# sydney-machine-learning/parallel-tempering-neural-net

Measured on AMD Instinct MI355X. Metric: MCMC samples/sec (all replicas) + swap-accept rate; Sunspot 64-replica FNN, higher is better.
Workload: dtype f32

## Files before the change

parallel-tempering-neural-net_amd/csrc/ptnn_dev_pack.hpp:

```cpp

constexpr int PK_WAVES = 8, PK_SWEEP_WAVES = 2, PK_FWD_WAVES = 4;
__host__ __device__ constexpr int pack_slots(int nred) { return PK_SWEEP_WAVES * (WAVE >> nred); }

__host__ __device__ inline size_t pack_slot_floats(int PS) { return 2 * (size_t)PS; }
__host__ __device__ inline size_t pack_ring_floats(int PS, int nslots) { return (size_t)2 * nslots * ((size_t)PS + 4); }
__host__ __device__ inline size_t pack_lds_floats(int Nall, int IPY, int PS, int H, int FWS, int nslots) {
    return (size_t)(Nall + 2) * IPY + 4 * (size_t)PS + MAX_WAVES * 8 + (size_t)nslots * SL_COUNT +
           (size_t)nslots * pack_slot_floats(PS) + pack_ring_floats(PS, nslots) + (size_t)PK_WAVES * fw_floats(H, FWS);
}
constexpr int PK_MULTI_MAXG = 4;
__host__ __device__ inline size_t pack_multi_lds_floats(int Nall, int IPY, int PS, int H, int FWS, int nslots) {
    return pack_lds_floats(Nall, IPY, PS, H, FWS, nslots) + pack_ring_floats(PS, (PK_MULTI_MAXG - 1) * nslots) + 2 * (size_t)PS + SL_COUNT + 8;
}

template <int TASK, int I, int O, int PK_NRED, bool MULTI = false>
__device__ __forceinline__ void segment_pack_body(const SegParams& p, const SegDyn& dyn, const int step_begin, const int n_steps) {
    constexpr int PK_NG = WAVE >> PK_NRED, PK_SLOTS = pack_slots(PK_NRED);
    extern __shared__ __attribute__((aligned(16))) float smem[];
    const int G = MULTI ? p.G : 1;
    const int lb = MULTI ? xcd_block(G) : (int)blockIdx.x;
    const int r = MULTI ? lb / G : lb, grp = MULTI ? lb - r * G : 0;
    const int KT = G * PK_SLOTS, s0 = grp * PK_SLOTS;
    const int gid = p.first_global + r;
    const int tid = threadIdx.x, nthr = blockDim.x;
    const int wave = tid >> 6, lane = tid & 63;
    const int Nall = p.Ntr + p.Nte;
    const int P = p.P, PS = p.PS, H = p.H;
    float* q = smem;
    float* xy = q; q += (Nall + 2) * p.IPY;
    float* w_cur = q; q += PS;
    float* w_gd = q; q += PS;
    float* rec_w = q; q += PS;
    float* rec_alt = q; q += PS;
    float* red = q; q += MAX_WAVES * 8;
    float* slots = q; q += PK_SLOTS * SL_COUNT;
    const size_t SLF = pack_slot_floats(PS);
    float* sl0 = q; q += PK_SLOTS * SLF;
    constexpr int RING = (MULTI ? 2 * PK_MULTI_MAXG : 2) * PK_SLOTS;
    float* ring_n = q; q += (size_t)RING * PS;
    float* ring_s = q; q += (size_t)RING * 4;
    float* my_fw = q + (size_t)wave * fw_floats(H, p.FWS);
    q += (size_t)PK_WAVES * fw_floats(H, p.FWS);
    float* win_v = q; q += MULTI ? 2 * (size_t)PS : 0;
    float* win_s = q; q += MULTI ? SL_COUNT : 0;
    float* gverd = q;
    granule_t* const xv = MULTI ? p.xverdict + (size_t)r * 2 * MAX_SLOTS : nullptr;
    granule_t* const xsl = MULTI ? p.xslots + (size_t)r * 2 * MAX_SLOTS * SL_COUNT : nullptr;
    granule_t* const xwv = MULTI ? p.xw + (size_t)r * 2 * G * 2 * PS : nullptr;
    unsigned epoch = dyn.epoch_base;
    int xpar = 0;
    bool failed = false;
    auto s_prop = [&](int s_) { return sl0 + (size_t)s_ * SLF; };
    auto s_pgd = [&](int s_) { return sl0 + (size_t)s_ * SLF + PS; };

    {
        const float4* src = reinterpret_cast<const float4*>(p.data);
        float4* dst = reinterpret_cast<float4*>(xy);
        for (int e = tid; e < ((Nall + 2) * p.IPY) >> 2; e += nthr) dst[e] = src[e];
    }
    float* gw = dyn.w_state + (size_t)r * PS;
    for (int j = tid; j < PS; j += nthr) {
        w_cur[j] = gw[j];
        rec_w[j] = p.rec_w[(size_t)r * PS + j];
        w_gd[j] = dyn.gd_w[(size_t)r * PS + j];
    }
    __syncthreads();

    const float T = uni_f(p.temps[r]);
    float eta = (TASK == TASK_REG) ? uni_f(w_cur[P]) : 0.0f;
    float* sf = p.st_f + (size_t)r * SF_COUNT;
    int* si = p.st_i + (size_t)r * SI_COUNT;
    float lik, prior_cur, tau_eta_last, rec_rmse_tr, rec_rmse_te, rec_acc_tr, rec_acc_te;
    int nacc, gd_valid, lg_count, lg_acc;
    if (step_begin == 0) {
        lg_acc = 0;
        if (wave == 0) {
            chain_startup<TASK, I, O, true>(p, xy, w_cur, my_fw, red, T, eta, lik, prior_cur);
            if (lane == 0) { red[0] = eta; red[1] = lik; red[2] = prior_cur; }
        }
        __syncthreads();
        eta = uni_f(red[0]); lik = uni_f(red[1]); prior_cur = uni_f(red[2]);
        tau_eta_last = eta;
        rec_rmse_tr = rec_rmse_te = rec_acc_tr = rec_acc_te = 0.f;
        nacc = 0; gd_valid = 0; lg_count = 0;
        __syncthreads();
    } else {
        lik = uni_f(sf[SF_LIK]); prior_cur = uni_f(sf[SF_PRIOR]); tau_eta_last = uni_f(sf[SF_TAU_LAST]);
        rec_rmse_tr = uni_f(sf[SF_REC_RMSE_TR]); rec_rmse_te = uni_f(sf[SF_REC_RMSE_TE]);
        rec_acc_tr = uni_f(sf[SF_REC_ACC_TR]); rec_acc_te = uni_f(sf[SF_REC_ACC_TE]);
        nacc = uni_i(si[SI_NACC]); gd_valid = uni_i(dyn.gd_valid[r]); lg_count = uni_i(si[SI_LG_COUNT]); lg_acc = uni_i(si[SI_LG_ACC]);
    }

    PTNN_DIAG(pack_begin);
    const size_t trow = (size_t)r * p.trace_cap;
    const int end = step_begin + n_steps;
    const bool sweeping = p.use_lg != 0;
    const int nwaves = nthr >> 6;
    const int ev_n = sweeping ? (nwaves == PK_WAVES ? PK_FWD_WAVES : 2) : nwaves;
    const int ev_i = !sweeping ? wave : ((wave & 3) >= 2 ? (wave & 1) + ((wave >> 2) << 1) : -1);
    int i = step_begin;
    int tpos0 = (step_begin + 1) % p.trace_cap;
    const float inv_PW = 1.0f / (float)p.PW;
    const int nq1 = ((P + 3) >> 2) + 1;
    auto fill_ring = [&](int lo, int hi, int wi, int nw) {
        if (nq1 <= WAVE) {
            const int per_pass = WAVE / nq1, ls = lane / nq1, q_ = lane - ls * nq1;
            for (int sb = lo + wi * per_pass; sb < hi; sb += nw * per_pass) {
                const int j = sb + ls;
                if (ls < per_pass && j < hi) {
                    const int slot = j % RING;
                    const bool sc = (q_ == nq1 - 1);
                    uint32_t x[4];
                    philox4x32_10(sc ? 0u : (uint32_t)q_, (uint32_t)j, p.noise_shared ? 0u : (uint32_t)gid, sc ? STREAM_STEP : STREAM_WNOISE,
                                  p.seed_lo, p.seed_hi, x);
                    float n0, n1, n2, n3;
                    box_muller(x[0], x[1], n0, n1);
                    box_muller(x[2], x[3], n2, n3);
                    if (sc) { float* sc_ = ring_s + slot * 4; sc_[0] = u23(x[0]); sc_[1] = u23(x[1]); sc_[2] = n2; }
                    else *reinterpret_cast<float4*>(ring_n + (size_t)slot * PS + 4 * q_) = make_float4(n0, n1, n2, n3);
                }
            }
        } else {
            for (int j = lo + wi; j < hi; j += nw) tape_step<true>(p, gid, j, ring_n + (size_t)(j % RING) * PS, ring_s + (j % RING) * 4);
        }
    };
    fill_ring(step_begin, step_begin + RING, wave, nwaves);
    int ring_hi = step_begin + RING;
    bool xcd_local = false;
    if constexpr (MULTI) {
        if (p.xcd_granules) xcd_local = xcd_handshake(xv + 32, G, grp, dyn.epoch_base, gverd);
    }
    __syncthreads();
    persist_cptr const pp = dyn.pp;
    const bool swap_inside = MULTI && pp->swap_inside != 0;
    const int si_ = pp->si;
    auto next_handoff = [&](int cur) {
        if (TASK == TASK_REG) { const int c1 = cur > 1 ? cur : 1; return ((c1 + si_ - 1) / si_) * si_; }
        return ((cur + si_) / si_) * si_ - 1;
    };
    int ho_next = swap_inside ? next_handoff(step_begin) : 0x7fffffff;
    int nx = 0;
    while (i < end && !failed) {
        if (MULTI) { epoch += 1; }
        if (i == p.switch_step) {
            if (wave == 0) {
                build_fw<I, O, true>(w_cur, my_fw, H, p.FWS);
                gsync<true>();
                const EvalSums sc = eval_rows<TASK, I, O, true>(my_fw, xy, p.IPY, p.FWS, H, p.Ntr, Nall, nullptr);
                float l2, r1, r2, a1, a2;
                finish_eval<TASK>(sc, p.Ntr, p.Nte, tau_eta_last, l2, r1, r2, a1, a2);
                if (lane == 0) red[0] = l2;
            }
            __syncthreads();
            lik = uni_f(red[0]);
            __syncthreads();
        }
        int kt = min(KT, end - i);
        if (p.switch_step > i) kt = min(kt, p.switch_step - i);
        if (swap_inside && ho_next >= i) kt = min(kt, ho_next - i + 1);
        const int k = MULTI ? max(0, min(PK_SLOTS, kt - s0)) : kt;
        PTNN_DIAG(count_round);
        STAMP(0);
        if (sweeping && !gd_valid) {
            if (wave == 0) sgd_sweep_dispatch<TASK, I, O>(w_cur, w_gd, xy, p.data, p.Ntr, H, p.lr);
            gd_valid = 1;
            __syncthreads();
        }
        const int rpos0 = (i + s0) % RING;
        auto s_noise = [&](int s_) { int e_ = rpos0 + s_; if (e_ >= RING) e_ -= RING; return ring_n + (size_t)e_ * PS; };
        auto s_scal = [&](int s_) { int e_ = rpos0 + s_; if (e_ >= RING) e_ -= RING; return ring_s + e_ * 4; };
        STAMP(1);
        STAMP(2);
        if (sweeping && wave < PK_SWEEP_WAVES) {
            const int ng = min(PK_NG, k - wave * PK_NG);
            if (ng > 0) {
                SweepProposals pp;
                pp.noise = ring_n; pp.scal = ring_s; pp.w_cur = w_cur; pp.w_gd = w_gd;
                pp.pos0 = rpos0 + wave * PK_NG; if (pp.pos0 >= RING) pp.pos0 -= RING;
                pp.ring = RING; pp.nstride = PS; pp.step_w = p.step_w; pp.l_prob = p.l_prob; pp.use_lg = 1;
                sgd_sweep<TASK, I, O, PK_NRED, true>(nullptr, s_pgd(wave * PK_NG), xy, p.data, p.Ntr, H, p.lr, ng, (int)SLF, &pp);
            }
        }
        STAMP(3);
        PTNN_DIAG(pack_eval_begin);
        if (ev_i >= 0) {
            for (int s_ = ev_i; s_ < k; s_ += ev_n) {
                const int j = i + s0 + s_;
                const float adapttemp = (p.switch_step >= 0 && j >= p.switch_step) ? 1.0f : T;
                const float* sc_ = s_scal(s_);
                const bool lg = sweeping && (sc_[0] < p.l_prob);
                float eta_pro = eta;
                if (TASK == TASK_REG) eta_pro = fmaf(p.step_eta, sc_[2], eta);
                {
                    const float* nz = s_noise(s_);
                    const float* base = lg ? w_gd : w_cur;
                    float* pr = s_prop(s_);
                    for (int e = lane; e < P; e += WAVE) pr[e] = fmaf(p.step_w, nz[e], base[e]);
                }
                gsync<true>();
                build_fw<I, O, true>(s_prop(s_), my_fw, H, p.FWS);
                gsync<true>();
                const EvalSums es = eval_rows<TASK, I, O, true>(my_fw, xy, p.IPY, p.FWS, H, p.Ntr, Nall, nullptr);
                float ll, rm_tr, rm_te, ac_tr, ac_te;
                finish_eval<TASK, true>(es, p.Ntr, p.Nte, eta_pro, ll, rm_tr, rm_te, ac_tr, ac_te);
                const float ssq = block_sumsq<true>(s_prop(s_), P, nullptr);
                const float prior_prop = prior_value<TASK>(p, ssq, eta_pro);
                const float d2 = lg ? block_sumsq<true>(s_noise(s_), P, nullptr) : 0.0f;
                if (lane == 0) {
                    float* sl = slots + s_ * SL_COUNT;
                    sl[SL_LIKPROP] = ll / adapttemp; sl[SL_PRIORPROP] = prior_prop; sl[SL_ETAPRO] = eta_pro;
                    sl[SL_RM_TR] = rm_tr; sl[SL_RM_TE] = rm_te; sl[SL_AC_TR] = ac_tr; sl[SL_AC_TE] = ac_te;
                    sl[SL_ADAPT] = adapttemp; sl[SL_LG] = lg ? 1.0f : 0.0f; sl[SL_D2] = d2;
                }
                gsync<true>();
            }
            fill_ring(ring_hi, i + RING, ev_i, ev_n);
        }
        ring_hi = i + RING;
        PTNN_DIAG(pack_eval_end);
        __syncthreads();
        STAMP(4);
        {
            const int s_ = wave * (WAVE / 16) + (lane >> 4), l16 = lane & 15;
            const bool on = s_ < k;
            float* sl = slots + (on ? s_ : 0) * SL_COUNT;
            float diff_prop = 0.0f;
            if (sweeping && wave < 4) {
                const float* pg = s_pgd(on ? s_ : 0);
                float r1[4];
#pragma unroll
                for (int c = 0; c < 4; ++c) {
                    float a1 = 0.0f;
                    for (int e = 16 * c + l16; e < P; e += WAVE) {
                        const float d = w_cur[e] - pg[e];
                        a1 = fmaf(d, d, a1);
                    }
                    r1[c] = (16 * c < P) ? group_allsum<4>(a1) : 0.0f;
                }
                const float d1 = (r1[0] + r1[1]) + (r1[2] + r1[3]);
                if (sl[SL_LG] != 0.0f) diff_prop = langevin_ratio(d1, sl[SL_D2], p.step_w, sl[SL_ADAPT]);
            }
            const float logalpha = (sl[SL_LIKPROP] - lik) + (sl[SL_PRIORPROP] - prior_cur) + diff_prop;
            const float mh = (logalpha != logalpha) ? 1.0f : fminf(1.0f, expf_fast(logalpha));
            if (on && l16 == 0) { sl[SL_ACCEPT] = (s_scal(s_)[1] < mh) ? 1.0f : 0.0f; sl[SL_LOGALPHA] = logalpha; }
        }
        __syncthreads();
        STAMP(5);
        const bool f_acc = (lane < k) && (slots[lane * SL_COUNT + SL_ACCEPT] != 0.0f);
        const unsigned long long bal_acc = __ballot(f_acc);
        const int ml = bal_acc ? (__ffsll((long long)bal_acc) - 1) : -1;
        int m = (ml >= 0) ? s0 + ml : kt;
        const float* sm = slots + (ml >= 0 ? ml : 0) * SL_COUNT;
        const float* wacc = s_prop(ml >= 0 ? ml : 0);
        if constexpr (MULTI) {
            granule_t* const xv_r = xv + (size_t)xpar * MAX_SLOTS;
            auto gstore = [&](granule_t* g_, float v_) { if (xcd_local) granule_store_xcd(g_, epoch, v_); else granule_store(g_, epoch, v_); };
            auto gwait = [&](const granule_t* g_, float& v_) { return xcd_local ? granule_wait_xcd(g_, epoch, v_) : granule_wait(g_, epoch, v_); };
            if (tid == 0) gstore(xv_r + grp, (float)ml);
            if (ml >= 0) {
                if (tid < SL_COUNT) gstore(xsl + ((size_t)xpar * MAX_SLOTS + grp) * SL_COUNT + tid, sm[tid]);
                granule_t* const xo = xwv + ((size_t)xpar * G + grp) * 2 * PS;
                for (int e = tid; e < 2 * PS; e += nthr) gstore(xo + e, wacc[e]);
            }
            if (tid < G) {
                float v = 0.0f;
                if (!gwait(xv_r + tid, v)) v = -2.0f;
                gverd[tid] = v;
            }
            __syncthreads();
            int win = -1;
            m = kt;
            for (int g_ = 0; g_ < G; ++g_) {
                const float v = gverd[g_];
                if (v == -2.0f) failed = true;
                const int cand = (v >= 0.0f) ? g_ * PK_SLOTS + (int)v : kt;
                if (cand < m) { m = cand; win = g_; }
            }
            if (failed) break;
            if (win >= 0 && win != grp) {
                bool ok = true;
                if (tid < SL_COUNT) {
                    float v;
                    ok = gwait(xsl + ((size_t)xpar * MAX_SLOTS + win) * SL_COUNT + tid, v);
                    win_s[tid] = v;
                }
                const granule_t* const xi = xwv + ((size_t)xpar * G + win) * 2 * PS;
                for (int e = tid; e < 2 * PS; e += nthr) {
                    float v;
                    ok = gwait(xi + e, v) && ok;
                    win_v[e] = v;
                }
                failed = __syncthreads_or(ok ? 0 : 1) != 0;
                if (failed) break;
                sm = win_s; wacc = win_v;
            }
            xpar ^= 1;
        }
        const int ncommit = (m < kt) ? m + 1 : kt;
        const int nloc = max(0, min(k, ncommit - s0));
        for (int item = tid; item < nloc * p.PW; item += nthr) {
            const int s_ = (int)(((float)item + 0.5f) * inv_PW), e = item - s_ * p.PW;
            int tp = tpos0 + s0 + s_;
            if (tp >= p.trace_cap) tp -= p.trace_cap;
            p.tr_pos_w[(trow + (size_t)tp) * (size_t)p.PW + e] = (e < P) ? ((s0 + s_ == m) ? s_prop(s_) : rec_w)[e] : 0.0f;
        }
        if (tid < nloc) {
            const int s_ = tid;
            const bool acc_me = (s0 + s_ == m);
            const float* sl = slots + s_ * SL_COUNT;
            int tp = tpos0 + s0 + s_;
            if (tp >= p.trace_cap) tp -= p.trace_cap;
            const size_t tpos = trow + (size_t)tp;
            store_trace_row(p.tr_scal + tpos * TR_COUNT, (TASK == TASK_REG) ? sl[SL_LIKPROP] : sl[SL_LIKPROP] * sl[SL_ADAPT],
                            acc_me ? sl[SL_RM_TR] : rec_rmse_tr, acc_me ? sl[SL_RM_TE] : rec_rmse_te,
                            acc_me ? sl[SL_AC_TR] : rec_acc_tr, acc_me ? sl[SL_AC_TE] : rec_acc_te, nacc, sl[SL_LOGALPHA]);
        }
        if constexpr (MULTI) {
            const int e_ = (i + lane) % RING;
            const bool f_lg = sweeping && (lane < ncommit) && (ring_s[e_ * 4] < p.l_prob);
            lg_count += __popcll(__ballot(f_lg));
            if (TASK == TASK_REG) tau_eta_last = uni_f(fmaf(p.step_eta, ring_s[((i + ncommit - 1) % RING) * 4 + 2], eta));
        } else {
            const bool f_lg = (lane < k) && (slots[lane * SL_COUNT + SL_LG] != 0.0f);
            const unsigned long long bal_lg = __ballot(f_lg);
            lg_count += __popcll(bal_lg & ((1ull << ncommit) - 1ull));
            if (TASK == TASK_REG) tau_eta_last = uni_f(slots[(ncommit - 1) * SL_COUNT + SL_ETAPRO]);
        }
        if (m < kt) {
            nacc += 1;
            lik = uni_f(sm[SL_LIKPROP]); prior_cur = uni_f(sm[SL_PRIORPROP]); eta = uni_f(sm[SL_ETAPRO]);
            rec_rmse_tr = uni_f(sm[SL_RM_TR]); rec_rmse_te = uni_f(sm[SL_RM_TE]);
            rec_acc_tr = uni_f(sm[SL_AC_TR]); rec_acc_te = uni_f(sm[SL_AC_TE]);
            lg_acc += (sm[SL_LG] != 0.0f) ? 1 : 0;
            gd_valid = sweeping ? 1 : 0;
            for (int e = tid; e < P; e += nthr) {
                const float v = wacc[e];
                w_cur[e] = v; rec_alt[e] = v;
                if (sweeping) w_gd[e] = wacc[PS + e];
            }
            float* t_ = rec_w; rec_w = rec_alt; rec_alt = t_;
        }
        __syncthreads();
        i += ncommit;
        tpos0 += ncommit;
        if (tpos0 >= p.trace_cap) tpos0 -= p.trace_cap;
        STAMP(6);
        if constexpr (MULTI) {
            if (swap_inside && i == ho_next + 1 && ho_next < end) {
                const int Rg = pp->sp.R, ROW = 2 * PS + 8;
                const unsigned xtag = dyn.epoch_base + (unsigned)nx + 1u;
                granule_t* const xl = p.xswap + (size_t)(nx & 1) * swap_xchg_granules(Rg, ROW);
                granule_t* const xst = xl + ((Rg + 7) & ~7);
                granule_t* const xsb = xst + (size_t)Rg * ROW + (size_t)gid * (ROW + 8);
                auto gstore = [&](granule_t* g_, float v_) { if (xcd_local) granule_store_xcd(g_, xtag, v_); else granule_store(g_, xtag, v_); };
                auto gwait = [&](const granule_t* g_, float& v_) { return xcd_local ? granule_wait_xcd(g_, xtag, v_) : granule_wait(g_, xtag, v_); };
                auto row_value = [&](int j) { return (j < PS) ? ((j == P) ? eta : ((j < P) ? w_cur[j] : 0.0f)) : ((j < 2 * PS) ? w_gd[j - PS] : ((j == 2 * PS) ? (gd_valid ? 1.0f : 0.0f) : 0.0f)); };
                auto row_take = [&](int j, float v) { if (j < PS) w_cur[j] = v; else if (j < 2 * PS) w_gd[j - PS] = v; else if (j == 2 * PS) red[1] = v; };
                bool ok = true;
                bool moved = false;
                if (grp == 0) {
                    if (tid == 0) granule_store(xl + gid, xtag, (TASK == TASK_REG) ? lik * T : lik);
                    for (int j = tid; j <= 2 * PS; j += nthr) granule_store(xst + (size_t)gid * ROW + j, xtag, row_value(j));
                    float* const sL = sl0;
                    float* const sU = sl0 + Rg;
                    int* const sSrc = reinterpret_cast<int*>(sl0 + 2 * Rg);
                    for (int k_ = tid; k_ < Rg; k_ += nthr) { float v = 0.0f; ok = granule_wait(xl + k_, xtag, v) && ok; sL[k_] = v; }
                    if (__syncthreads_or(ok ? 0 : 1)) { failed = true; break; }
#if defined(__HIP_DEVICE_COMPILE__)
                    const SwapParams sp = pp->sp;
#else
                    const SwapParams sp{};
#endif
                    const int round = pp->round0 + nx;
                    const int nsw = cascade_lds(sp, round, sL, sU, sSrc, true);
                    const int src = sSrc[gid];
                    if (gid == sp.first_global) {
                        if (sp.src_log && round < sp.log_capacity)
                            for (int k_ = tid; k_ < Rg; k_ += nthr) sp.src_log[(size_t)round * Rg + k_] = sSrc[k_];
                        if (tid == 0) { sp.counters[0] += nsw; sp.counters[1] += Rg - 1; }
                    }
                    __syncthreads();
                    moved = src != gid;
                    if (moved) {
                        for (int j = tid; j <= 2 * PS; j += nthr) { float v = 0.0f; ok = granule_wait(xst + (size_t)src * ROW + j, xtag, v) && ok; row_take(j, v); }
                        if (__syncthreads_or(ok ? 0 : 1)) { failed = true; break; }
                        for (int j = tid; j <= 2 * PS; j += nthr) gstore(xsb + 8 + j, (j == 2 * PS) ? red[1] : ((j < PS) ? w_cur[j] : w_gd[j - PS]));
                    }
                    if (tid == 0) gstore(xsb, moved ? 1.0f : 0.0f);
                } else {
                    if (tid == 0) { float mv = 0.0f; ok = gwait(xsb, mv); red[0] = mv; }
                    if (__syncthreads_or(ok ? 0 : 1)) { failed = true; break; }
                    moved = red[0] != 0.0f;
                    if (moved) {
                        for (int j = tid; j <= 2 * PS; j += nthr) { float v = 0.0f; ok = gwait(xsb + 8 + j, v) && ok; row_take(j, v); }
                        if (__syncthreads_or(ok ? 0 : 1)) { failed = true; break; }
                    }
                }
                __syncthreads();
                if (moved) {
                    if (TASK == TASK_REG) eta = uni_f(w_cur[P]);
                    gd_valid = (uni_f(red[1]) != 0.0f) ? 1 : 0;
                }
                __syncthreads();
                nx += 1;
                ho_next = next_handoff(i);
            }
        }
    }
    PTNN_DIAG(pack_flush);

    if (failed) {
        if (tid == 0) atomicAdd(p.error_flag, 1);
        return;
    }
    if (grp != 0) return;
    const int fl_end = (pp->flip0 + nx) & 1;
    float* const gw_end = swap_inside ? pp->state[fl_end] + (size_t)r * PS : gw;
    float* const gd_end = swap_inside ? pp->gd[fl_end] + (size_t)r * PS : dyn.gd_w + (size_t)r * PS;
    int* const gdv_end = swap_inside ? pp->gd_valid[fl_end] : dyn.gd_valid;
    for (int j = tid; j < PS; j += nthr) {
        gw_end[j] = (j == P) ? eta : w_cur[j];
        p.rec_w[(size_t)r * PS + j] = rec_w[j];
        gd_end[j] = w_gd[j];
    }
    if (tid == 0) {
        sf[SF_LIK] = lik; sf[SF_PRIOR] = prior_cur; sf[SF_TAU_LAST] = tau_eta_last;
        sf[SF_REC_RMSE_TR] = rec_rmse_tr; sf[SF_REC_RMSE_TE] = rec_rmse_te;
        sf[SF_REC_ACC_TR] = rec_acc_tr; sf[SF_REC_ACC_TE] = rec_acc_te;
        si[SI_NACC] = nacc; gdv_end[r] = gd_valid; si[SI_LG_COUNT] = lg_count; si[SI_LG_ACC] = lg_acc;
        p.L_handoff[gid] = (TASK == TASK_REG) ? lik * T : lik;
        p.L_final[gid] = lik;
        post_raw(p, gid, lik, prior_cur, T, step_begin + n_steps - 1);
    }
}
```

Before: 15.63 million.

## Pipeline sweep and forward-eval waves with LDS flag handshakes and double-buffered slots

Adds a pipelined path for the single-group sweeping case. The sweep waves (gradient proposals plus MH accept decisions) and the forward-eval waves run decoupled, synchronising through LDS atomic counters and flags instead of block-wide barriers. Slot buffers are double-buffered so sweep waves can build the next round's proposals from the speculatively accepted state while eval waves commit the trace. This removes per-round __syncthreads stalls, at the cost of doubled LDS for the slots and more complex spin-wait logic that can time out or deadlock.

```diff
diff --git a/parallel-tempering-neural-net_amd/csrc/ptnn_dev_pack.hpp b/parallel-tempering-neural-net_amd/csrc/ptnn_dev_pack.hpp
--- a/parallel-tempering-neural-net_amd/csrc/ptnn_dev_pack.hpp
+++ b/parallel-tempering-neural-net_amd/csrc/ptnn_dev_pack.hpp
@@ -4,13 +4,20 @@
 
 __host__ __device__ inline size_t pack_slot_floats(int PS) { return 2 * (size_t)PS; }
 __host__ __device__ inline size_t pack_ring_floats(int PS, int nslots) { return (size_t)2 * nslots * ((size_t)PS + 4); }
+constexpr int PK_SYNC = 8;
 __host__ __device__ inline size_t pack_lds_floats(int Nall, int IPY, int PS, int H, int FWS, int nslots) {
-    return (size_t)(Nall + 2) * IPY + 4 * (size_t)PS + MAX_WAVES * 8 + (size_t)nslots * SL_COUNT +
-           (size_t)nslots * pack_slot_floats(PS) + pack_ring_floats(PS, nslots) + (size_t)PK_WAVES * fw_floats(H, FWS);
+    return (size_t)(Nall + 2) * IPY + 4 * (size_t)PS + MAX_WAVES * 8 + 2 * (size_t)nslots * SL_COUNT +
+           2 * (size_t)nslots * pack_slot_floats(PS) + pack_ring_floats(PS, nslots) + (size_t)PK_WAVES * fw_floats(H, FWS) + PK_SYNC;
 }
 constexpr int PK_MULTI_MAXG = 4;
 __host__ __device__ inline size_t pack_multi_lds_floats(int Nall, int IPY, int PS, int H, int FWS, int nslots) {
     return pack_lds_floats(Nall, IPY, PS, H, FWS, nslots) + pack_ring_floats(PS, (PK_MULTI_MAXG - 1) * nslots) + 2 * (size_t)PS + SL_COUNT + 8;
+}
+
+__device__ __forceinline__ int opaque_lane(int lane) {
+    int l;
+    asm volatile("v_mov_b32 %0, %1" : "=v"(l) : "v"(lane));
+    return l;
 }
 
 template <int TASK, int I, int O, int PK_NRED, bool MULTI = false>
@@ -30,12 +37,15 @@
     float* xy = q; q += (Nall + 2) * p.IPY;
     float* w_cur = q; q += PS;
     float* w_gd = q; q += PS;
-    float* rec_w = q; q += PS;
-    float* rec_alt = q; q += PS;
+    float* const rec_a = q; q += PS;
+    float* const rec_b = q; q += PS;
+    float* rec_w = rec_a;
+    float* rec_alt = rec_b;
     float* red = q; q += MAX_WAVES * 8;
-    float* slots = q; q += PK_SLOTS * SL_COUNT;
+    float* slots = q; q += 2 * PK_SLOTS * SL_COUNT;
     const size_t SLF = pack_slot_floats(PS);
-    float* sl0 = q; q += PK_SLOTS * SLF;
+    float* sl0 = q; q += 2 * PK_SLOTS * SLF;
+    unsigned* const psync = reinterpret_cast<unsigned*>(q); q += PK_SYNC;
     constexpr int RING = (MULTI ? 2 * PK_MULTI_MAXG : 2) * PK_SLOTS;
     float* ring_n = q; q += (size_t)RING * PS;
     float* ring_s = q; q += (size_t)RING * 4;
@@ -64,6 +74,7 @@
         rec_w[j] = p.rec_w[(size_t)r * PS + j];
         w_gd[j] = dyn.gd_w[(size_t)r * PS + j];
     }
+    if (tid < PK_SYNC) psync[tid] = 0u;
     __syncthreads();
 
     const float T = uni_f(p.temps[r]);
@@ -98,6 +109,7 @@
     const int nwaves = nthr >> 6;
     const int ev_n = sweeping ? (nwaves == PK_WAVES ? PK_FWD_WAVES : 2) : nwaves;
     const int ev_i = !sweeping ? wave : ((wave & 3) >= 2 ? (wave & 1) + ((wave >> 2) << 1) : -1);
+    const bool pipelined = !MULTI && sweeping && nwaves == PK_WAVES;
     int i = step_begin;
     int tpos0 = (step_begin + 1) % p.trace_cap;
     const float inv_PW = 1.0f / (float)p.PW;
@@ -165,6 +177,221 @@
             if (wave == 0) sgd_sweep_dispatch<TASK, I, O>(w_cur, w_gd, xy, p.data, p.Ntr, H, p.lr);
             gd_valid = 1;
             __syncthreads();
+        }
+        if constexpr (!MULTI) {
+            if (pipelined) {
+                const int seg_end = (p.switch_step > i) ? min(end, p.switch_step) : end;
+                int bofs = -1;
+                int par = 0;
+                unsigned wn = 0;
+                auto lds_wait = [&](const unsigned* w_, unsigned want, bool ge, unsigned& v_) {
+                    for (unsigned spins = 0; spins < SPIN_LIMIT; ++spins) {
+                        v_ = uni_i((int)__hip_atomic_load(w_, __ATOMIC_ACQUIRE, __HIP_MEMORY_SCOPE_WORKGROUP));
+                        if (ge ? v_ >= want : (v_ >> 16) == want) return true;
+                        __builtin_amdgcn_s_sleep(1);
+                    }
+                    return false;
+                };
+                if (wave < PK_SWEEP_WAVES) {
+                    while (true) {
+                        const int kt = min(KT, seg_end - i);
+                        float* const SLs = slots + par * PK_SLOTS * SL_COUNT;
+                        float* const SV = sl0 + (size_t)par * PK_SLOTS * SLF;
+                        const int rpos0 = i % RING;
+                        if (wn > 0) { PTNN_DIAG(count_round); }
+                        STAMP(0);
+                        const float* const bc = bofs < 0 ? w_cur : sl0 + bofs;
+                        const int ng = min(PK_NG, kt - wave * PK_NG);
+                        if (ng > 0) {
+                            SweepProposals pp;
+                            pp.noise = ring_n; pp.scal = ring_s; pp.w_cur = bc; pp.w_gd = bofs < 0 ? w_gd : bc + PS;
+                            pp.pos0 = rpos0 + wave * PK_NG; if (pp.pos0 >= RING) pp.pos0 -= RING;
+                            pp.ring = RING; pp.nstride = PS; pp.step_w = p.step_w; pp.l_prob = p.l_prob; pp.use_lg = 1;
+                            sgd_sweep<TASK, I, O, PK_NRED, true>(nullptr, SV + (size_t)wave * PK_NG * SLF + PS, xy, p.data, p.Ntr, H, p.lr,
+                                                                 ng, (int)SLF, &pp);
+                        }
+                        STAMP(3);
+                        unsigned v_ = 0;
+                        if (!lds_wait(psync, (unsigned)PK_FWD_WAVES * (wn + 1u), true, v_)) failed = true;
+                        STAMP(4);
+                        const int ln = opaque_lane(lane);
+                        unsigned mask = 0;
+#pragma unroll
+                        for (int h = 0; h < PK_NG / 4; ++h) {
+                            const int s_ = wave * PK_NG + h * 4 + (ln >> 4), l16 = ln & 15;
+                            const bool on = s_ < kt;
+                            float* sl = SLs + (on ? s_ : 0) * SL_COUNT;
+                            const float* pg = SV + (size_t)(on ? s_ : 0) * SLF + PS;
+                            float r1[4];
+#pragma unroll
+                            for (int c = 0; c < 4; ++c) {
+                                float a1 = 0.0f;
+                                for (int e = 16 * c + l16; e < P; e += WAVE) {
+                                    const float d = bc[e] - pg[e];
+                                    a1 = fmaf(d, d, a1);
+                                }
+                                r1[c] = (16 * c < P) ? group_allsum<4>(a1) : 0.0f;
+                            }
+                            const float d1 = (r1[0] + r1[1]) + (r1[2] + r1[3]);
+                            bool acc = false;
+                            if (on) {
+                                if (sl[SL_LG] != 0.0f) {
+                                    const float diff_prop = langevin_ratio(d1, sl[SL_D2], p.step_w, sl[SL_ADAPT]);
+                                    const float logalpha = sl[SL_LOGALPHA] + diff_prop;
+                                    const float mh = (logalpha != logalpha) ? 1.0f : fminf(1.0f, expf_fast(logalpha));
+                                    int e_ = rpos0 + s_; if (e_ >= RING) e_ -= RING;
+                                    acc = ring_s[e_ * 4 + 1] < mh;
+                                    if (l16 == 0) sl[SL_LOGALPHA] = logalpha;
+                                } else {
+                                    acc = sl[SL_ACCEPT] != 0.0f;
+                                }
+                            }
+                            const unsigned long long b = __ballot(acc && l16 == 0);
+                            mask |= (unsigned)((b & 1ull) | ((b >> 15) & 2ull) | ((b >> 30) & 4ull) | ((b >> 45) & 8ull)) << (4 * h);
+                        }
+                        if (ln == 0)
+                            __hip_atomic_store(psync + 1 + 2 * wave + par, ((wn + 1u) << 16) | mask, __ATOMIC_RELEASE, __HIP_MEMORY_SCOPE_WORKGROUP);
+                        unsigned full = mask << (wave * PK_NG);
+                        if (wave != 0 || mask == 0) {
+                            const int o = 1 - wave;
+                            if (!lds_wait(psync + 1 + 2 * o + par, wn + 1u, false, v_)) failed = true;
+                            full |= (v_ & 0xffffu) << (o * PK_NG);
+                        }
+                        const int m = full ? __builtin_ctz(full) : kt;
+                        bofs = (m < kt) ? (par * PK_SLOTS + m) * (int)SLF : -1;
+                        i += (m < kt) ? m + 1 : kt;
+                        par ^= 1;
+                        wn += 1;
+                        STAMP(5);
+                        if (i >= seg_end || failed) break;
+                    }
+                } else if (ev_i >= 0) {
+                    const int nft = PK_FWD_WAVES * WAVE;
+                    while (true) {
+                        const int kt = min(KT, seg_end - i);
+                        float* const SLs = slots + par * PK_SLOTS * SL_COUNT;
+                        float* const SV = sl0 + (size_t)par * PK_SLOTS * SLF;
+                        const int rpos0 = i % RING;
+                        const float* const bc = bofs < 0 ? w_cur : sl0 + bofs;
+                        const float* const bg = bofs < 0 ? w_gd : bc + PS;
+                        const int ln = opaque_lane(lane), ft = ev_i * WAVE + ln;
+                        PTNN_DIAG(pack_eval_begin);
+                        for (int s_ = ev_i; s_ < kt; s_ += PK_FWD_WAVES) {
+                            const int j = i + s_;
+                            const float adapttemp = (p.switch_step >= 0 && j >= p.switch_step) ? 1.0f : T;
+                            int e_ = rpos0 + s_; if (e_ >= RING) e_ -= RING;
+                            const float* sc_ = ring_s + e_ * 4;
+                            const float* nz = ring_n + (size_t)e_ * PS;
+                            const bool lg = sc_[0] < p.l_prob;
+                            float eta_pro = eta;
+                            if (TASK == TASK_REG) eta_pro = fmaf(p.step_eta, sc_[2], eta);
+                            float* pr = SV + (size_t)s_ * SLF;
+                            {
+                                const float* base = lg ? bg : bc;
+                                for (int e = ln; e < P; e += WAVE) pr[e] = fmaf(p.step_w, nz[e], base[e]);
+                            }
+                            gsync<true>();
+                            build_fw<I, O, true>(pr, my_fw, H, p.FWS);
+                            gsync<true>();
+                            const EvalSums es = eval_rows<TASK, I, O, true>(my_fw, xy, p.IPY, p.FWS, H, p.Ntr, Nall, nullptr);
+                            float ll, rm_tr, rm_te, ac_tr, ac_te;
+                            finish_eval<TASK, true>(es, p.Ntr, p.Nte, eta_pro, ll, rm_tr, rm_te, ac_tr, ac_te);
+                            const float ssq = block_sumsq<true>(pr, P, nullptr);
+                            const float prior_prop = prior_value<TASK>(p, ssq, eta_pro);
+                            const float d2 = lg ? block_sumsq<true>(nz, P, nullptr) : 0.0f;
+                            if (ln == 0) {
+                                float* sl = SLs + s_ * SL_COUNT;
+                                const float likprop = ll / adapttemp;
+                                sl[SL_LIKPROP] = likprop; sl[SL_PRIORPROP] = prior_prop; sl[SL_ETAPRO] = eta_pro;
+                                sl[SL_RM_TR] = rm_tr; sl[SL_RM_TE] = rm_te; sl[SL_AC_TR] = ac_tr; sl[SL_AC_TE] = ac_te;
+                                sl[SL_ADAPT] = adapttemp; sl[SL_LG] = lg ? 1.0f : 0.0f; sl[SL_D2] = d2;
+                                const float la = (likprop - lik) + (prior_prop - prior_cur);
+                                if (lg) {
+                                    sl[SL_LOGALPHA] = la;
+                                } else {
+                                    const float diff_prop = 0.0f;
+                                    const float logalpha = la + diff_prop;
+                                    const float mh = (logalpha != logalpha) ? 1.0f : fminf(1.0f, expf_fast(logalpha));
+                                    sl[SL_ACCEPT] = (sc_[1] < mh) ? 1.0f : 0.0f; sl[SL_LOGALPHA] = logalpha;
+                                }
+                            }
+                            gsync<true>();
+                        }
+                        fill_ring(ring_hi, i + RING, ev_i, PK_FWD_WAVES);
+                        ring_hi = i + RING;
+                        PTNN_DIAG(pack_eval_end);
+                        if (ln == 0) __hip_atomic_fetch_add(psync, 1u, __ATOMIC_RELEASE, __HIP_MEMORY_SCOPE_WORKGROUP);
+                        unsigned v0 = 0, v1 = 0;
+                        if (!lds_wait(psync + 1 + par, wn + 1u, false, v0)) failed = true;
+                        if (!failed && (v0 & 0xffffu) == 0 && !lds_wait(psync + 3 + par, wn + 1u, false, v1)) failed = true;
+                        if (failed) break;
+                        const unsigned full = (v0 & 0xffffu) | ((v1 & 0xffffu) << PK_NG);
+                        const int m = full ? __builtin_ctz(full) : kt;
+                        const int ncommit = (m < kt) ? m + 1 : kt;
+                        const float* const wacc = SV + (size_t)(m < kt ? m : 0) * SLF;
+                        for (int item = ft; item < ncommit * p.PW; item += nft) {
+                            const int s_ = (int)(((float)item + 0.5f) * inv_PW), e = item - s_ * p.PW;
+                            int tp = tpos0 + s_;
+                            if (tp >= p.trace_cap) tp -= p.trace_cap;
+                            p.tr_pos_w[(trow + (size_t)tp) * (size_t)p.PW + e] = (e < P) ? ((s_ == m) ? wacc : rec_w)[e] : 0.0f;
+                        }
+                        if (ft < ncommit) {
+                            const int s_ = ft;
+                            const bool acc_me = (s_ == m);
+                            const float* sl = SLs + s_ * SL_COUNT;
+                            int tp = tpos0 + s_;
+                            if (tp >= p.trace_cap) tp -= p.trace_cap;
+                            const size_t tpos = trow + (size_t)tp;
+                            store_trace_row(p.tr_scal + tpos * TR_COUNT, (TASK == TASK_REG) ? sl[SL_LIKPROP] : sl[SL_LIKPROP] * sl[SL_ADAPT],
+                                            acc_me ? sl[SL_RM_TR] : rec_rmse_tr, acc_me ? sl[SL_RM_TE] : rec_rmse_te,
+                                            acc_me ? sl[SL_AC_TR] : rec_acc_tr, acc_me ? sl[SL_AC_TE] : rec_acc_te, nacc, sl[SL_LOGALPHA]);
+                        }
+                        const bool f_lg = (ln < kt) && (SLs[ln * SL_COUNT + SL_LG] != 0.0f);
+                        lg_count += __popcll(__ballot(f_lg) & ((1ull << ncommit) - 1ull));
+                        if (TASK == TASK_REG) tau_eta_last = uni_f(SLs[(ncommit - 1) * SL_COUNT + SL_ETAPRO]);
+                        if (m < kt) {
+                            const float* sm = SLs + m * SL_COUNT;
+                            nacc += 1;
+                            lik = uni_f(sm[SL_LIKPROP]); prior_cur = uni_f(sm[SL_PRIORPROP]); eta = uni_f(sm[SL_ETAPRO]);
+                            rec_rmse_tr = uni_f(sm[SL_RM_TR]); rec_rmse_te = uni_f(sm[SL_RM_TE]);
+                            rec_acc_tr = uni_f(sm[SL_AC_TR]); rec_acc_te = uni_f(sm[SL_AC_TE]);
+                            lg_acc += (sm[SL_LG] != 0.0f) ? 1 : 0;
+                            for (int e = ft; e < P; e += nft) {
+                                const float v = wacc[e];
+                                w_cur[e] = v; rec_alt[e] = v;
+                                w_gd[e] = wacc[PS + e];
+                            }
+                            float* t_ = rec_w; rec_w = rec_alt; rec_alt = t_;
+                        }
+                        bofs = (m < kt) ? (par * PK_SLOTS + m) * (int)SLF : -1;
+                        i += ncommit;
+                        tpos0 += ncommit;
+                        if (tpos0 >= p.trace_cap) tpos0 -= p.trace_cap;
+                        par ^= 1;
+                        wn += 1;
+                        if (i >= seg_end) break;
+                    }
+                }
+                failed = __syncthreads_or(failed ? 1 : 0) != 0;
+                float* const bcast = red + 32;
+                if (wave == 2 && lane == 0) {
+                    bcast[0] = lik; bcast[1] = prior_cur; bcast[2] = eta; bcast[3] = tau_eta_last;
+                    bcast[4] = rec_rmse_tr; bcast[5] = rec_rmse_te; bcast[6] = rec_acc_tr; bcast[7] = rec_acc_te;
+                    bcast[8] = __int_as_float(nacc); bcast[9] = __int_as_float(lg_count); bcast[10] = __int_as_float(lg_acc);
+                    bcast[11] = __int_as_float(i); bcast[12] = __int_as_float(tpos0); bcast[13] = __int_as_float(ring_hi);
+                    bcast[14] = __int_as_float(rec_w == rec_a ? 0 : 1);
+                }
+                if (tid < PK_SYNC) psync[tid] = 0u;
+                __syncthreads();
+                lik = uni_f(bcast[0]); prior_cur = uni_f(bcast[1]); eta = uni_f(bcast[2]); tau_eta_last = uni_f(bcast[3]);
+                rec_rmse_tr = uni_f(bcast[4]); rec_rmse_te = uni_f(bcast[5]); rec_acc_tr = uni_f(bcast[6]); rec_acc_te = uni_f(bcast[7]);
+                nacc = uni_i(__float_as_int(bcast[8])); lg_count = uni_i(__float_as_int(bcast[9])); lg_acc = uni_i(__float_as_int(bcast[10]));
+                i = uni_i(__float_as_int(bcast[11])); tpos0 = uni_i(__float_as_int(bcast[12])); ring_hi = uni_i(__float_as_int(bcast[13]));
+                const bool sw_ = uni_i(__float_as_int(bcast[14])) != 0;
+                rec_w = sw_ ? rec_b : rec_a; rec_alt = sw_ ? rec_a : rec_b;
+                STAMP(6);
+                continue;
+            }
         }
         const int rpos0 = (i + s0) % RING;
         auto s_noise = [&](int s_) { int e_ = rpos0 + s_; if (e_ >= RING) e_ -= RING; return ring_n + (size_t)e_ * PS; };
```

After: 15.76 million (median of 6 runs). Within noise of the previous version (+0.8%).
